# fdaPDE/fdaPDE-core

Hardware: AMD Instinct MI355X
Metric: DOF/s assemble+solve, 3D P1 Laplacian; SpMV achieved HBM GB/s vs peak (higher is better)
Workload: dtype f64

## Files before the change

fdapde-core_amd/csrc/dev_persist.hip:

```cpp
#include <hip/hip_runtime.h>
#include <hipcub/hipcub.hpp>

#include <algorithm>
#include <chrono>
#include <cstdint>
#include <string>
#include <vector>

#include "dev_persist.h"

namespace fdapde_hip {

namespace {

#define DP_CHK(expr)                                                          \
    do {                                                                      \
        hipError_t e__ = (expr);                                              \
        if (e__ != hipSuccess) {                                              \
            err = std::string(#expr) + ": " + hipGetErrorString(e__);         \
            return FDAPDE_EHIP;                                               \
        }                                                                     \
    } while (0)

struct Arena {
    std::vector<void*> slabs;
    char* cur = nullptr;
    size_t left = 0;
    static constexpr size_t kSlab = size_t(768) << 20;
    hipError_t take(size_t bytes, void** out) {
        bytes = (bytes + 255) & ~size_t(255);
        if (bytes > left) {
            const size_t sz = bytes > kSlab ? bytes : kSlab;
            void* p = nullptr;
            const hipError_t e = hipMalloc(&p, sz);
            if (e != hipSuccess) return e;
            slabs.push_back(p), cur = static_cast<char*>(p), left = sz;
        }
        *out = cur, cur += bytes, left -= bytes;
        return hipSuccess;
    }
    ~Arena() {
        for (void* p : slabs) (void)hipFree(p);
    }
};
thread_local Arena* t_arena = nullptr;
struct ArenaScope {
    Arena* prev;
    explicit ArenaScope(Arena* a) : prev(t_arena) { t_arena = a; }
    ~ArenaScope() { t_arena = prev; }
};
template <typename T> struct Tmp {
    T* p = nullptr;
    size_t n = 0;
    bool own = false;
    hipError_t alloc(size_t count) {
        reset();
        n = count;
        if (t_arena) return t_arena->take(sizeof(T) * (count ? count : 1), reinterpret_cast<void**>(&p));
        own = true;
        return hipMalloc(reinterpret_cast<void**>(&p), sizeof(T) * (count ? count : 1));
    }
    void reset() {
        if (p && own) (void)hipFree(p);
        p = nullptr, n = 0, own = false;
    }
    ~Tmp() { reset(); }
};
struct Scratch {
    void* p = nullptr;
    size_t n = 0;
    hipError_t need(size_t bytes) {
        if (bytes <= n) return hipSuccess;
        if (p) (void)hipFree(p);
        n = bytes + bytes / 4;
        return hipMalloc(&p, n);
    }
    ~Scratch() {
        if (p) (void)hipFree(p);
    }
};
inline unsigned grid_of(int64_t n) { return (unsigned)((n + 255) / 256); }

__device__ __forceinline__ int32_t wg_of_irow(const int32_t* wgs, int G, int64_t i) {
    int lo = 0, hi = G;
    while (hi - lo > 1) {
        const int mid = (lo + hi) >> 1;
        if (wgs[mid] <= i) lo = mid; else hi = mid;
    }
    return lo;
}
__global__ void k_balance_bounds(int G, int64_t nd, int64_t total, const int32_t* len_scan, const int32_t* irow_scan, int32_t* wgs) {
    const int g = blockIdx.x * blockDim.x + threadIdx.x;
    if (g > G) return;
    if (g == G) {
        wgs[G] = irow_scan[nd];
        return;
    }
    const int64_t target = (int64_t)g * total / G;
    int64_t lo = 0, hi = nd;
    while (lo < hi) {
        const int64_t mid = (lo + hi) >> 1;
        if ((int64_t)len_scan[mid] + 2 * (int64_t)irow_scan[mid] >= target) hi = mid; else lo = mid + 1;
    }
    wgs[g] = irow_scan[lo];
}
__global__ void k_wg_of(int64_t nd, const uint8_t* keep, const int32_t* irow, const int32_t* wgs, int G, int32_t* wg) {
    const int64_t d = (int64_t)blockIdx.x * blockDim.x + threadIdx.x;
    if (d < nd) wg[d] = keep[d] ? wg_of_irow(wgs, G, irow[d]) : -1;
}
__device__ __forceinline__ bool kept_entry(const uint8_t* keep, int32_t row, int32_t col) { return col != row && keep[col]; }

__global__ void k_keep_flags(int64_t nd, const uint8_t* bnd, int use_bnd, uint8_t* keep, int32_t* keep32) {
    const int64_t d = (int64_t)blockIdx.x * blockDim.x + threadIdx.x;
    if (d >= nd) return;
    const uint8_t k = (use_bnd && bnd[d]) ? 0 : 1;
    keep[d] = k, keep32[d] = k;
}
__global__ void k_row_lengths(int64_t nd, const int32_t* rowptr, const int32_t* colidx, const uint8_t* keep, int32_t* len) {
    const int64_t d = (int64_t)blockIdx.x * blockDim.x + threadIdx.x;
    if (d >= nd) return;
    int32_t n = 0;
    if (keep[d])
        for (int32_t k = rowptr[d]; k < rowptr[d + 1]; ++k) n += kept_entry(keep, (int32_t)d, colidx[k]);
    len[d] = n;
}
__global__ void k_sym_own_init(int64_t nd, const int32_t* rowptr, const int32_t* colidx, const uint8_t* keep, int32_t* own, const int32_t* irow,
                               int32_t* kept_dof) {
    const int64_t d = (int64_t)blockIdx.x * blockDim.x + threadIdx.x;
    if (d >= nd || !keep[d]) return;
    if (kept_dof) kept_dof[irow[d]] = (int32_t)d;
    for (int32_t k = rowptr[d]; k < rowptr[d + 1]; ++k) own[k] = persist_sym_owner((int32_t)d, colidx[k]) ? 1 : 0;
}
__global__ void k_sym_rows(int64_t nd, const int32_t* rowptr, const int32_t* colidx, const uint8_t* keep, const int32_t* wg, const int32_t* irow,
                           const int32_t* wgs, const int32_t* own, uint8_t* par, int32_t* up_k, int32_t* up_m, int32_t* up_loc) {
    const int64_t d = (int64_t)blockIdx.x * blockDim.x + threadIdx.x;
    if (d >= nd || !keep[d]) return;
    const int32_t g = wg[d], i = irow[d];
    int32_t len = 0, k_up = -1;
    for (int32_t k = rowptr[d]; k < rowptr[d + 1]; ++k) {
        const int32_t c = colidx[k];
        if (!kept_entry(keep, (int32_t)d, c)) continue;
        const bool inb = wg[c] == g;
        len += (!inb || own[k] != 0) ? 1 : 0;
        if (inb && c > (int32_t)d && k_up < 0) k_up = k;
    }
    par[i] = (uint8_t)(len & 1), up_k[i] = k_up;
    int32_t km = -1, loc = -1;
    if (k_up >= 0) {
        const int32_t c = colidx[k_up];
        int32_t lo = rowptr[c], hi = rowptr[c + 1];
        while (lo < hi) {
            const int32_t mid = (lo + hi) >> 1;
            if (colidx[mid] < (int32_t)d) lo = mid + 1; else hi = mid;
        }
        km = lo, loc = irow[c] - wgs[g];
    }
    up_m[i] = km, up_loc[i] = loc;
}
__global__ __launch_bounds__(256) void k_sym_walk(const int32_t* wgs, const uint8_t* par_g, const int32_t* up_k, const int32_t* up_m, const int32_t* up_loc,
                                                  int32_t* own) {
    extern __shared__ int32_t sw_lds[];
    const int g = blockIdx.x;
    const int32_t i0 = wgs[g], rows = wgs[g + 1] - i0;
    int32_t* up = sw_lds;
    uint8_t* par = reinterpret_cast<uint8_t*>(sw_lds + rows);
    for (int32_t i = threadIdx.x; i < rows; i += blockDim.x) up[i] = up_loc[i0 + i], par[i] = par_g[i0 + i];
    __syncthreads();
    if (threadIdx.x == 0)
        for (int32_t i = 0; i < rows; ++i) {
            const int32_t u = up[i];
            if ((par[i] & 1) && u >= 0) par[i] = 2, par[u] ^= 1;
        }
    __syncthreads();
    for (int32_t i = threadIdx.x; i < rows; i += blockDim.x)
        if (par[i] & 2) {
            const int32_t ku = up_k[i0 + i], km = up_m[i0 + i];
            own[ku] ^= 1, own[km] ^= 1;
        }
}
__global__ void k_row_lengths_sym(int64_t nd, const int32_t* rowptr, const int32_t* colidx, const uint8_t* keep, const int32_t* wg, const int32_t* own,
                                  int32_t* len) {
    const int64_t d = (int64_t)blockIdx.x * blockDim.x + threadIdx.x;
    if (d >= nd) return;
    int32_t n = 0;
    if (keep[d]) {
        const int32_t g = wg[d];
        for (int32_t k = rowptr[d]; k < rowptr[d + 1]; ++k) {
            const int32_t c = colidx[k];
            n += kept_entry(keep, (int32_t)d, c) && (wg[c] != g || own[k] != 0);
        }
    }
    len[d] = n;
}
__device__ __forceinline__ void wave_count_by_key(bool flag, int32_t key, int32_t* cnt) {
    unsigned long long todo = __ballot(flag);
    const int lane = (int)(threadIdx.x & 63);
    while (todo) {
        const int leader = __ffsll((long long)todo) - 1;
        const int32_t k0 = __shfl(key, leader);
        const unsigned long long same = __ballot(flag && key == k0);
        if (lane == leader) atomicAdd(&cnt[k0], (int32_t)__popcll(same));
        todo &= ~same;
    }
}
__global__ void k_row_halo(int64_t nd, const int32_t* rowptr, const int32_t* colidx, const uint8_t* keep, const int32_t* wg,
                           uint8_t* halo, int32_t* n_out, int32_t* wg_halo) {
    const int64_t d = (int64_t)blockIdx.x * blockDim.x + threadIdx.x;
    int32_t n = 0, g = -1;
    if (d < nd && keep[d]) {
        g = wg[d];
        for (int32_t k = rowptr[d]; k < rowptr[d + 1]; ++k) {
            const int32_t c = colidx[k];
            n += kept_entry(keep, (int32_t)d, c) && wg[c] != g;
        }
    }
    wave_count_by_key(n != 0, g, wg_halo);
    if (d < nd) halo[d] = n ? 1 : 0, n_out[d] = n;
}
__global__ void k_import_pairs(int64_t nd, const int32_t* rowptr, const int32_t* colidx, const uint8_t* keep, const int32_t* wg,
                               const int32_t* at, uint64_t* key) {
    const int64_t d = (int64_t)blockIdx.x * blockDim.x + threadIdx.x;
    if (d >= nd || !keep[d]) return;
    const int32_t g = wg[d];
    int32_t o = at[d];
    for (int32_t k = rowptr[d]; k < rowptr[d + 1]; ++k) {
        const int32_t c = colidx[k];
        if (kept_entry(keep, (int32_t)d, c) && wg[c] != g) key[o++] = ((uint64_t)(uint32_t)g << 32) | (uint32_t)c;
    }
}
__global__ void k_unique_flags(int64_t n, const uint64_t* key, int32_t* flag) {
    const int64_t i = (int64_t)blockIdx.x * blockDim.x + threadIdx.x;
    if (i < n) flag[i] = (i == 0 || key[i] != key[i - 1]) ? 1 : 0;
}
__global__ void k_compact_keys(int64_t n, const uint64_t* key, const int32_t* flag, const int32_t* pos, uint64_t* out) {
    const int64_t i = (int64_t)blockIdx.x * blockDim.x + threadIdx.x;
    if (i < n && flag[i]) out[pos[i]] = key[i];
}
__global__ void k_row_keys1(int64_t nd, const uint8_t* keep, const int32_t* irow, const int32_t* wg, const uint8_t* halo, const int32_t* len,
                            uint64_t* key, int32_t* val) {
    const int64_t d = (int64_t)blockIdx.x * blockDim.x + threadIdx.x;
    if (d >= nd || !keep[d]) return;
    const int32_t i = irow[d];
    key[i] = ((uint64_t)(uint32_t)wg[d] << 41) | ((uint64_t)halo[d] << 40) | ((uint64_t)(255 - len[d]) << 32) | (uint32_t)d;
    val[i] = (int32_t)d;
}
__global__ void k_row_keys2(int64_t n_int, const int32_t* dof_sorted, const int32_t* wgs, int G, int32_t sa, const uint8_t* halo, const int32_t* len,
                            uint64_t* key) {
    const int64_t p = (int64_t)blockIdx.x * blockDim.x + threadIdx.x;
    if (p >= n_int) return;
    const int32_t d = dof_sorted[p];
    const int64_t g = wg_of_irow(wgs, G, p), rank = p - wgs[g];
    const bool first = !halo[d] && rank < sa;
    const uint64_t payload = first ? (uint64_t)rank : (((uint64_t)(255 - len[d]) << 33) | ((uint64_t)halo[d] << 32) | (uint32_t)d);
    key[p] = ((uint64_t)g << 42) | ((uint64_t)(first ? 0 : 1) << 41) | payload;
}
__global__ void k_assign_slots(int64_t n_int, const int32_t* dof_sorted, const int32_t* wgs, int G, int32_t sa, int32_t S, const int32_t* wg_noimp, int32_t* slot_of,
                               int32_t* slot_dof) {
    const int64_t p = (int64_t)blockIdx.x * blockDim.x + threadIdx.x;
    if (p >= n_int) return;
    const int32_t d = dof_sorted[p];
    const int64_t g = wg_of_irow(wgs, G, p), i = p - wgs[g];
    const int32_t n_a = min(wg_noimp[g], sa);
    const int32_t slot = i < n_a ? (int32_t)i : sa + (int32_t)(i - n_a);
    slot_of[d] = slot;
    slot_dof[g * S + slot] = d;
}
__global__ void k_mark_exports(int64_t n_imp, const uint64_t* imp_key, uint8_t* is_exp) {
    const int64_t i = (int64_t)blockIdx.x * blockDim.x + threadIdx.x;
    if (i < n_imp) is_exp[imp_key[i] & 0xffffffffu] = 1;
}
__global__ void k_export_keys(int64_t nd, const uint8_t* is_exp, const int32_t* wg, const int32_t* slot_of, uint64_t* key, int32_t* val,
                              int32_t* n_out, int32_t* wg_exp) {
    const int64_t d = (int64_t)blockIdx.x * blockDim.x + threadIdx.x;
    const bool e = d < nd && is_exp[d];
    const int32_t g = e ? wg[d] : -1;
    const unsigned long long m = __ballot(e);
    if (m == 0) return;
    const int lane = (int)(threadIdx.x & 63), leader = __ffsll((long long)m) - 1;
    int32_t base = 0;
    if (lane == leader) base = atomicAdd(n_out, (int32_t)__popcll(m));
    base = __shfl(base, leader);
    if (e) {
        const int32_t o = base + (int32_t)__popcll(m & ((1ull << lane) - 1ull));
        key[o] = ((uint64_t)(uint32_t)g << 32) | (uint32_t)slot_of[d];
        val[o] = (int32_t)d;
    }
    wave_count_by_key(e, g, wg_exp);
}
__global__ void k_board_tables(int64_t n_board, const uint64_t* key_sorted, const int32_t* dof_sorted, uint16_t* exp_slot, int32_t* board_of) {
    const int64_t i = (int64_t)blockIdx.x * blockDim.x + threadIdx.x;
    if (i >= n_board) return;
    exp_slot[i] = (uint16_t)(key_sorted[i] & 0xffffu);
    board_of[dof_sorted[i]] = (int32_t)i;
}
__global__ void k_import_board_keys(int64_t n_imp, const uint64_t* imp_key, const int32_t* board_of, uint64_t* key, int32_t* wg_imp) {
    const int64_t i = (int64_t)blockIdx.x * blockDim.x + threadIdx.x;
    const bool in = i < n_imp;
    const uint64_t g = in ? imp_key[i] >> 32 : 0;
    if (in) key[i] = (g << 32) | (uint32_t)board_of[imp_key[i] & 0xffffffffu];
    wave_count_by_key(in, (int32_t)g, wg_imp);
}
__global__ void k_count_groups(int64_t n, const uint64_t* key, int32_t* count) {
    const int64_t i = (int64_t)blockIdx.x * blockDim.x + threadIdx.x;
    wave_count_by_key(i < n, i < n ? (int32_t)(key[i] >> 32) : 0, count);
}
__global__ void k_low32(int64_t n, const uint64_t* key, int32_t* out) {
    const int64_t i = (int64_t)blockIdx.x * blockDim.x + threadIdx.x;
    if (i < n) out[i] = (int32_t)(key[i] & 0xffffffffu);
}
__global__ void k_slice_pairs(int64_t n_sl, const int32_t* slot_dof, const int32_t* len, int32_t* pairs) {
    const int64_t q = (int64_t)blockIdx.x * blockDim.x + threadIdx.x;
    if (q >= n_sl) return;
    int32_t w = 0;
    for (int l = 0; l < 64; ++l) {
        const int32_t d = slot_dof[q * 64 + l];
        if (d >= 0) w = max(w, len[d]);
    }
    pairs[q] = (w + 1) / 2;
}
__global__ void k_slice_offsets(int G, int nsl, const int32_t* scan, int32_t* sl_off, int64_t* ell_off, int32_t* max_block) {
    const int64_t t = (int64_t)blockIdx.x * blockDim.x + threadIdx.x;
    if (t >= (int64_t)G * (nsl + 1)) return;
    const int64_t g = t / (nsl + 1), q = t - g * (nsl + 1);
    const int32_t base = scan[g * nsl];
    sl_off[t] = scan[g * nsl + q] - base;
    if (q == nsl) atomicMax(max_block, scan[g * nsl + nsl] - base);
    if (q == 0) ell_off[g] = (int64_t)base * 128;
    if (t == 0) ell_off[G] = (int64_t)scan[(int64_t)G * nsl] * 128;
}
__global__ void k_fill_ell(int64_t n_slots, int32_t S, int nsl, const int32_t* slot_dof, const int32_t* rowptr, const int32_t* colidx, const uint8_t* keep,
                           const int32_t* wg, const int32_t* slot_of, const int32_t* board_of, const int32_t* imp_off,
                           const int32_t* imp_pos, const int32_t* sl_off, const int64_t* ell_off, int sym, const int32_t* own, uint16_t* code, int32_t* src) {
    const int64_t t = (int64_t)blockIdx.x * blockDim.x + threadIdx.x;
    if (t >= n_slots) return;
    const int32_t d = slot_dof[t];
    if (d < 0 && !sym) return;
    const int64_t g = t / S;
    const int32_t s = (int32_t)(t - g * S), q = s / 64, l = s % 64;
    const int64_t base = ell_off[g] + (int64_t)sl_off[g * (nsl + 1) + q] * 128 + 2 * l;
    int32_t e = 0;
    for (int32_t k = d < 0 ? 0 : rowptr[d]; k < (d < 0 ? 0 : rowptr[d + 1]); ++k) {
        const int32_t c = colidx[k];
        if (!kept_entry(keep, d, c)) continue;
        if (sym && wg[c] == (int32_t)g && own[k] == 0) continue;
        const int64_t at = base + (int64_t)(e / 2) * 128 + (e & 1);
        src[at] = k;
        if (wg[c] == (int32_t)g) {
            code[at] = (uint16_t)slot_of[c];
        } else {
            int32_t lo = imp_off[g], hi = imp_off[g + 1];
            const int32_t b = board_of ? board_of[c] : c;
            while (lo < hi) {
                const int32_t mid = (lo + hi) >> 1;
                if (imp_pos[mid] < b) lo = mid + 1; else hi = mid;
            }
            code[at] = (uint16_t)(S + (lo - imp_off[g]));
        }
        ++e;
    }
    if (sym) {
        const int32_t e1 = 2 * (sl_off[g * (nsl + 1) + q + 1] - sl_off[g * (nsl + 1) + q]);
        for (; e < e1; ++e) code[base + (int64_t)(e / 2) * 128 + (e & 1)] = (uint16_t)s;
    }
}
__global__ void k_drop_list(int64_t nd, const uint8_t* keep, const int32_t* irow_scan, int32_t* drop) {
    const int64_t d = (int64_t)blockIdx.x * blockDim.x + threadIdx.x;
    if (d < nd && !keep[d]) drop[d - irow_scan[d]] = (int32_t)d;
}
__global__ void k_scatter_irow(int64_t nd, const uint8_t* keep, const int32_t* irow_scan, int32_t* irow) {
    const int64_t d = (int64_t)blockIdx.x * blockDim.x + threadIdx.x;
    if (d < nd) irow[d] = keep[d] ? irow_scan[d] : -1 - irow_scan[d];
}

template <typename K, typename V>
int sort_pairs(Scratch& sc, K* k_in, K* k_out, V* v_in, V* v_out, int64_t n, int end_bit, hipStream_t st, std::string& err) {
    size_t need = 0;
    DP_CHK(hipcub::DeviceRadixSort::SortPairs(nullptr, need, k_in, k_out, v_in, v_out, (int)n, 0, end_bit, st));
    DP_CHK(sc.need(need));
    DP_CHK(hipcub::DeviceRadixSort::SortPairs(sc.p, need, k_in, k_out, v_in, v_out, (int)n, 0, end_bit, st));
    return FDAPDE_OK;
}
template <typename K> int sort_keys(Scratch& sc, K* k_in, K* k_out, int64_t n, int end_bit, hipStream_t st, std::string& err) {
    size_t need = 0;
    DP_CHK(hipcub::DeviceRadixSort::SortKeys(nullptr, need, k_in, k_out, (int)n, 0, end_bit, st));
    DP_CHK(sc.need(need));
    DP_CHK(hipcub::DeviceRadixSort::SortKeys(sc.p, need, k_in, k_out, (int)n, 0, end_bit, st));
    return FDAPDE_OK;
}
template <typename In, typename Out> int exclusive_sum(Scratch& sc, In* in, Out* out, int64_t n, hipStream_t st, std::string& err) {
    size_t need = 0;
    DP_CHK(hipcub::DeviceScan::ExclusiveSum(nullptr, need, in, out, (int)n, st));
    DP_CHK(sc.need(need));
    DP_CHK(hipcub::DeviceScan::ExclusiveSum(sc.p, need, in, out, (int)n, st));
    return FDAPDE_OK;
}

}

void dev_persist_release(DevPersist* p) {
    if (!p) return;
    for (void* q : {(void*)p->slot_dof, (void*)p->sl_off, (void*)p->ell_src, (void*)p->exp_off, (void*)p->imp_off, (void*)p->imp_pos, (void*)p->ell_off,
                    (void*)p->ell_code, (void*)p->exp_slot, (void*)p->drop_dof})
        if (q) (void)hipFree(q);
    *p = DevPersist{};
}

int dev_build_persist_layout(int64_t nd, int32_t max_row, const int32_t* d_rowptr, const int32_t* d_colidx, const uint8_t* d_bnd, bool use_bnd,
                             int n_wg, int lds_entries, int blocked_rows, const int32_t* block_rows, int sym_mode, bool balance, void* stream, PersistLayout& pl, DevPersist* out,
                             std::string& err) {
    constexpr int T = kPersistT;
    hipStream_t st = static_cast<hipStream_t>(stream);
    if (n_wg < 1 || nd < 1 || max_row > 255) return FDAPDE_EUNSUPPORTED;
    const bool blocked = blocked_rows > 0;
    if (!blocked && n_wg > T) n_wg = T;
    Arena arena;
    ArenaScope arena_scope(&arena);
    Scratch sc;
    DevPersist o;
    struct Guard {
        DevPersist* p;
        bool armed = true;
        ~Guard() {
            if (armed) dev_persist_release(p);
        }
    } guard{&o};
    const bool dbg = std::getenv("FDAPDE_DEBUG_SETUP") != nullptr;
    auto t_ph = std::chrono::steady_clock::now();
    auto phase = [&](const char* name) {
        if (!dbg) return;
        (void)hipStreamSynchronize(st);
        const auto now = std::chrono::steady_clock::now();
        std::fprintf(stderr, "persist layout %-26s %8.2f ms\n", name, std::chrono::duration<double, std::milli>(now - t_ph).count());
        t_ph = now;
    };
    Tmp<uint8_t> keep, halo, is_exp;
    Tmp<int32_t> keep32, irow_scan, irow, len, n_imp_row, imp_at, wg_cnt;
    DP_CHK(keep.alloc((size_t)nd));
    DP_CHK(keep32.alloc((size_t)nd + 1));
    DP_CHK(irow_scan.alloc((size_t)nd + 1));
    DP_CHK(irow.alloc((size_t)nd));
    DP_CHK(len.alloc((size_t)nd + 1));
    DP_CHK(hipMemsetAsync(keep32.p + nd, 0, sizeof(int32_t), st));
    hipLaunchKernelGGL(k_keep_flags, dim3(grid_of(nd)), dim3(256), 0, st, nd, d_bnd, use_bnd ? 1 : 0, keep.p, keep32.p);
    if (int rc = exclusive_sum(sc, keep32.p, irow_scan.p, nd + 1, st, err)) return rc;
    hipLaunchKernelGGL(k_scatter_irow, dim3(grid_of(nd)), dim3(256), 0, st, nd, keep.p, irow_scan.p, irow.p);
    DP_CHK(hipMemsetAsync(len.p + nd, 0, sizeof(int32_t), st));
    hipLaunchKernelGGL(k_row_lengths, dim3(grid_of(nd)), dim3(256), 0, st, nd, d_rowptr, d_colidx, keep.p, len.p);
    Tmp<int32_t> len_scan;
    DP_CHK(len_scan.alloc((size_t)nd + 1));
    if (int rc = exclusive_sum(sc, len.p, len_scan.p, nd + 1, st, err)) return rc;
    int32_t h_nint = 0, h_nnz = 0;
    DP_CHK(hipMemcpyAsync(&h_nint, irow_scan.p + nd, sizeof(int32_t), hipMemcpyDeviceToHost, st));
    DP_CHK(hipMemcpyAsync(&h_nnz, len_scan.p + nd, sizeof(int32_t), hipMemcpyDeviceToHost, st));
    DP_CHK(hipStreamSynchronize(st));
    const int64_t n_int = h_nint, nnz_kept = h_nnz;
    if (n_int < 1) return FDAPDE_EUNSUPPORTED;
    const int64_t want = persist_want_workgroups(n_int, nnz_kept, lds_entries, blocked ? 0 : pl.single_rows);
    int G = (int)std::min<int64_t>(n_wg, want);
    if (blocked) G = (int)((n_int + blocked_rows - 1) / blocked_rows);
    if (G < 1) G = 1;
    if (G >= (1 << 20)) return FDAPDE_EUNSUPPORTED;
    int64_t rpw = (n_int + G - 1) / G;
    if (!blocked && block_rows == nullptr && rpw > (int64_t)kPersistRwide * T) return FDAPDE_EUNSUPPORTED;
    const bool sym = !blocked && persist_want_sym(sym_mode, nnz_kept, G, rpw) && rpw <= (int64_t)kPersistRmax * T;
    std::vector<int32_t> h_wgs;
    Tmp<int32_t> wgs, wg;
    bool uniform = true;
    if (block_rows != nullptr && !blocked) {
        G = n_wg;
        h_wgs.assign((size_t)G + 1, 0);
        rpw = 0;
        for (int g = 0; g < G; ++g) h_wgs[(size_t)g + 1] = h_wgs[(size_t)g] + block_rows[g], rpw = std::max<int64_t>(rpw, block_rows[g]);
        if (h_wgs[(size_t)G] != n_int) return FDAPDE_EINVAL;
        uniform = false;
    } else {
        G = (int)((n_int + rpw - 1) / rpw);
        DP_CHK(wgs.alloc((size_t)G + 1));
        if (balance && !blocked && G >= 2) {
            hipLaunchKernelGGL(k_balance_bounds, dim3((G + 256) / 256), dim3(256), 0, st, G, nd, nnz_kept + 2 * n_int, len_scan.p, irow_scan.p, wgs.p);
            h_wgs.assign((size_t)G + 1, 0);
            DP_CHK(hipMemcpyAsync(h_wgs.data(), wgs.p, sizeof(int32_t) * ((size_t)G + 1), hipMemcpyDeviceToHost, st));
            DP_CHK(hipStreamSynchronize(st));
            uniform = false;
            int64_t mx = 0;
            for (int g = 0; g < G; ++g) {
                if (h_wgs[(size_t)g + 1] <= h_wgs[(size_t)g]) uniform = true;
                mx = std::max<int64_t>(mx, h_wgs[(size_t)g + 1] - h_wgs[(size_t)g]);
            }
            const int64_t cap_rows = (int64_t)(rpw <= (int64_t)kPersistRmax * T ? kPersistRmax : kPersistRwide) * T;
            if (mx > cap_rows && rpw <= cap_rows) uniform = true;
            if (!uniform) rpw = mx;
        }
        if (uniform) {
            h_wgs.assign((size_t)G + 1, 0);
            for (int g = 0; g <= G; ++g) h_wgs[(size_t)g] = (int32_t)std::min<int64_t>(n_int, (int64_t)g * rpw);
        }
    }
    if (block_rows != nullptr && !blocked) DP_CHK(wgs.alloc((size_t)G + 1));
    DP_CHK(wg.alloc((size_t)nd));
    if (uniform || block_rows != nullptr) DP_CHK(hipMemcpyAsync(wgs.p, h_wgs.data(), sizeof(int32_t) * ((size_t)G + 1), hipMemcpyHostToDevice, st));
    hipLaunchKernelGGL(k_wg_of, dim3(grid_of(nd)), dim3(256), 0, st, nd, keep.p, irow.p, wgs.p, G, wg.p);
    phase("rows, workgroups");
    int64_t nnz_stored = nnz_kept;
    Tmp<int32_t> own;
    if (sym) {
        int32_t h_nnz_full = 0;
        DP_CHK(hipMemcpyAsync(&h_nnz_full, d_rowptr + nd, sizeof(int32_t), hipMemcpyDeviceToHost, st));
        DP_CHK(hipStreamSynchronize(st));
        DP_CHK(own.alloc((size_t)(h_nnz_full > 0 ? h_nnz_full : 1)));
        hipLaunchKernelGGL(k_sym_own_init, dim3(grid_of(nd)), dim3(256), 0, st, nd, d_rowptr, d_colidx, keep.p, own.p, irow.p, (int32_t*)nullptr);
        {
            Tmp<uint8_t> par;
            Tmp<int32_t> up_k, up_m, up_loc;
            DP_CHK(par.alloc((size_t)n_int));
            DP_CHK(up_k.alloc((size_t)n_int));
            DP_CHK(up_m.alloc((size_t)n_int));
            DP_CHK(up_loc.alloc((size_t)n_int));
            hipLaunchKernelGGL(k_sym_rows, dim3(grid_of(nd)), dim3(256), 0, st, nd, d_rowptr, d_colidx, keep.p, wg.p, irow.p, wgs.p, own.p, par.p, up_k.p, up_m.p,
                               up_loc.p);
            const size_t lds = (size_t)rpw * 5 + 16;
            hipLaunchKernelGGL(k_sym_walk, dim3(G), dim3(256), lds, st, wgs.p, par.p, up_k.p, up_m.p, up_loc.p, own.p);
            DP_CHK(hipGetLastError());
            if (!t_arena) DP_CHK(hipStreamSynchronize(st));
        }
        hipLaunchKernelGGL(k_row_lengths_sym, dim3(grid_of(nd)), dim3(256), 0, st, nd, d_rowptr, d_colidx, keep.p, wg.p, own.p, len.p);
        if (int rc = exclusive_sum(sc, len.p, len_scan.p, nd + 1, st, err)) return rc;
        DP_CHK(hipMemcpyAsync(&h_nnz, len_scan.p + nd, sizeof(int32_t), hipMemcpyDeviceToHost, st));
        DP_CHK(hipStreamSynchronize(st));
        nnz_stored = h_nnz;
    }
    phase("pair ownership (sym)");
    pl.n_drop = nd - n_int, pl.sym = sym;
    if (blocked) {
        DP_CHK(hipMalloc(reinterpret_cast<void**>(&o.drop_dof), sizeof(int32_t) * (size_t)(pl.n_drop ? pl.n_drop : 1)));
        hipLaunchKernelGGL(k_drop_list, dim3(grid_of(nd)), dim3(256), 0, st, nd, keep.p, irow_scan.p, o.drop_dof);
    }
    DP_CHK(halo.alloc((size_t)nd));
    DP_CHK(n_imp_row.alloc((size_t)nd + 1));
    DP_CHK(imp_at.alloc((size_t)nd + 1));
    DP_CHK(wg_cnt.alloc((size_t)3 * G));
    DP_CHK(hipMemsetAsync(wg_cnt.p, 0, sizeof(int32_t) * 3 * (size_t)G, st));
    DP_CHK(hipMemsetAsync(n_imp_row.p + nd, 0, sizeof(int32_t), st));
    hipLaunchKernelGGL(k_row_halo, dim3(grid_of(nd)), dim3(256), 0, st, nd, d_rowptr, d_colidx, keep.p, wg.p, halo.p, n_imp_row.p, wg_cnt.p);
    if (int rc = exclusive_sum(sc, n_imp_row.p, imp_at.p, nd + 1, st, err)) return rc;
    int32_t h_pairs = 0;
    std::vector<int32_t> h_cnt(3 * (size_t)G);
    DP_CHK(hipMemcpyAsync(&h_pairs, imp_at.p + nd, sizeof(int32_t), hipMemcpyDeviceToHost, st));
    DP_CHK(hipMemcpyAsync(h_cnt.data(), wg_cnt.p, sizeof(int32_t) * (size_t)G, hipMemcpyDeviceToHost, st));
    DP_CHK(hipStreamSynchronize(st));
    int32_t max_halo = 0;
    for (int g = 0; g < G; ++g) max_halo = std::max(max_halo, h_cnt[(size_t)g]);
    const int R = persist_rows_per_thread(rpw, max_halo, blocked, sym);
    if (R == 0) return FDAPDE_EUNSUPPORTED;
    const int S = R * T, nsl = S / 64, SA = blocked ? S : (R / 2) * T;
    pl.G = G, pl.R = R, pl.nsl = nsl, pl.n_int = n_int, pl.nnz = nnz_stored, pl.nnz_full = nnz_kept;
    Tmp<uint64_t> imp_key;
    int64_t n_imp = 0;
    {
        Tmp<uint64_t> k_a, k_s;
        Tmp<int32_t> flag, pos;
        DP_CHK(k_a.alloc((size_t)h_pairs));
        DP_CHK(k_s.alloc((size_t)h_pairs));
        DP_CHK(flag.alloc((size_t)h_pairs + 1));
        DP_CHK(pos.alloc((size_t)h_pairs + 1));
        hipLaunchKernelGGL(k_import_pairs, dim3(grid_of(nd)), dim3(256), 0, st, nd, d_rowptr, d_colidx, keep.p, wg.p, imp_at.p, k_a.p);
        if (h_pairs > 0) {
            if (int rc = sort_keys(sc, k_a.p, k_s.p, h_pairs, 53, st, err)) return rc;
            DP_CHK(hipMemsetAsync(flag.p + h_pairs, 0, sizeof(int32_t), st));
            hipLaunchKernelGGL(k_unique_flags, dim3(grid_of(h_pairs)), dim3(256), 0, st, (int64_t)h_pairs, k_s.p, flag.p);
            if (int rc = exclusive_sum(sc, flag.p, pos.p, (int64_t)h_pairs + 1, st, err)) return rc;
            int32_t h_n = 0;
            DP_CHK(hipMemcpyAsync(&h_n, pos.p + h_pairs, sizeof(int32_t), hipMemcpyDeviceToHost, st));
            DP_CHK(hipStreamSynchronize(st));
            n_imp = h_n;
            DP_CHK(imp_key.alloc((size_t)n_imp));
            hipLaunchKernelGGL(k_compact_keys, dim3(grid_of(h_pairs)), dim3(256), 0, st, (int64_t)h_pairs, k_s.p, flag.p, pos.p, imp_key.p);
            DP_CHK(hipStreamSynchronize(st));
        }
    }
    phase("import pairs");
    Tmp<int32_t> slot_of, dof1, wg_noimp;
    DP_CHK(slot_of.alloc((size_t)nd));
    DP_CHK(dof1.alloc((size_t)n_int));
    DP_CHK(hipMalloc(reinterpret_cast<void**>(&o.slot_dof), sizeof(int32_t) * (size_t)G * S));
    DP_CHK(hipMemsetAsync(o.slot_dof, 0xff, sizeof(int32_t) * (size_t)G * S, st));
    {
        Tmp<uint64_t> k_a, k_s;
        Tmp<int32_t> v_a, v_s;
        DP_CHK(k_a.alloc((size_t)n_int));
        DP_CHK(k_s.alloc((size_t)n_int));
        DP_CHK(v_a.alloc((size_t)n_int));
        DP_CHK(v_s.alloc((size_t)n_int));
        hipLaunchKernelGGL(k_row_keys1, dim3(grid_of(nd)), dim3(256), 0, st, nd, keep.p, irow.p, wg.p, halo.p, len.p, k_a.p, v_a.p);
        if (int rc = sort_pairs(sc, k_a.p, k_s.p, v_a.p, v_s.p, n_int, 62, st, err)) return rc;
        hipLaunchKernelGGL(k_row_keys2, dim3(grid_of(n_int)), dim3(256), 0, st, n_int, v_s.p, wgs.p, G, (int32_t)SA, halo.p, len.p, k_a.p);
        if (int rc = sort_pairs(sc, k_a.p, k_s.p, v_s.p, dof1.p, n_int, 63, st, err)) return rc;
        std::vector<int32_t> h_noimp((size_t)G);
        for (int g = 0; g < G; ++g)
            h_noimp[(size_t)g] = (h_wgs[(size_t)g + 1] - h_wgs[(size_t)g]) - (blocked ? 0 : h_cnt[(size_t)g]);
        DP_CHK(wg_noimp.alloc((size_t)G));
        DP_CHK(hipMemcpyAsync(wg_noimp.p, h_noimp.data(), sizeof(int32_t) * (size_t)G, hipMemcpyHostToDevice, st));
        hipLaunchKernelGGL(k_assign_slots, dim3(grid_of(n_int)), dim3(256), 0, st, n_int, dof1.p, wgs.p, G, (int32_t)SA, (int32_t)S, wg_noimp.p, slot_of.p,
                           o.slot_dof);
        DP_CHK(hipStreamSynchronize(st));
    }
    phase("slots");
    Tmp<int32_t> board_of;
    DP_CHK(board_of.alloc((size_t)nd));
    DP_CHK(is_exp.alloc((size_t)nd));
    DP_CHK(hipMemsetAsync(is_exp.p, 0, (size_t)nd, st));
    if (n_imp > 0 && !blocked) hipLaunchKernelGGL(k_mark_exports, dim3(grid_of(n_imp)), dim3(256), 0, st, n_imp, imp_key.p, is_exp.p);
    int64_t n_board = 0;
    if (!blocked) {
        Tmp<uint64_t> k_a, k_s;
        Tmp<int32_t> v_a, v_s, cnt;
        const int64_t cap = n_imp > 0 ? n_imp : 1;
        DP_CHK(k_a.alloc((size_t)cap));
        DP_CHK(k_s.alloc((size_t)cap));
        DP_CHK(v_a.alloc((size_t)cap));
        DP_CHK(v_s.alloc((size_t)cap));
        DP_CHK(cnt.alloc(1));
        DP_CHK(hipMemsetAsync(cnt.p, 0, sizeof(int32_t), st));
        hipLaunchKernelGGL(k_export_keys, dim3(grid_of(nd)), dim3(256), 0, st, nd, is_exp.p, wg.p, slot_of.p, k_a.p, v_a.p, cnt.p, wg_cnt.p + G);
        int32_t h_nb = 0;
        DP_CHK(hipMemcpyAsync(&h_nb, cnt.p, sizeof(int32_t), hipMemcpyDeviceToHost, st));
        DP_CHK(hipStreamSynchronize(st));
        n_board = h_nb;
        DP_CHK(hipMalloc(reinterpret_cast<void**>(&o.exp_slot), sizeof(uint16_t) * (size_t)(n_board ? n_board : 1)));
        if (n_board > 0) {
            if (int rc = sort_pairs(sc, k_a.p, k_s.p, v_a.p, v_s.p, n_board, 42, st, err)) return rc;
            hipLaunchKernelGGL(k_board_tables, dim3(grid_of(n_board)), dim3(256), 0, st, n_board, k_s.p, v_s.p, o.exp_slot, board_of.p);
        }
        DP_CHK(hipStreamSynchronize(st));
    }
    DP_CHK(hipMalloc(reinterpret_cast<void**>(&o.imp_pos), sizeof(int32_t) * (size_t)(n_imp ? n_imp : 1)));
    if (blocked) {
        DP_CHK(hipMalloc(reinterpret_cast<void**>(&o.exp_slot), sizeof(uint16_t)));
        if (n_imp > 0) {
            hipLaunchKernelGGL(k_low32, dim3(grid_of(n_imp)), dim3(256), 0, st, n_imp, imp_key.p, o.imp_pos);
            hipLaunchKernelGGL(k_count_groups, dim3(grid_of(n_imp)), dim3(256), 0, st, n_imp, imp_key.p, wg_cnt.p + 2 * G);
        }
    } else if (n_imp > 0) {
        Tmp<uint64_t> k_a, k_s;
        DP_CHK(k_a.alloc((size_t)n_imp));
        DP_CHK(k_s.alloc((size_t)n_imp));
        hipLaunchKernelGGL(k_import_board_keys, dim3(grid_of(n_imp)), dim3(256), 0, st, n_imp, imp_key.p, board_of.p, k_a.p, wg_cnt.p + 2 * G);
        if (int rc = sort_keys(sc, k_a.p, k_s.p, n_imp, 42, st, err)) return rc;
        hipLaunchKernelGGL(k_low32, dim3(grid_of(n_imp)), dim3(256), 0, st, n_imp, k_s.p, o.imp_pos);
        DP_CHK(hipStreamSynchronize(st));
    }
    DP_CHK(hipMemcpyAsync(h_cnt.data() + G, wg_cnt.p + G, sizeof(int32_t) * 2 * (size_t)G, hipMemcpyDeviceToHost, st));
    DP_CHK(hipStreamSynchronize(st));
    std::vector<int32_t> h_exp_off((size_t)G + 1, 0), h_imp_off((size_t)G + 1, 0);
    pl.max_exp = pl.max_imp = 0;
    for (int g = 0; g < G; ++g) {
        h_exp_off[(size_t)g + 1] = h_exp_off[(size_t)g] + h_cnt[(size_t)G + g], pl.max_exp = std::max(pl.max_exp, h_cnt[(size_t)G + g]);
        h_imp_off[(size_t)g + 1] = h_imp_off[(size_t)g] + h_cnt[(size_t)2 * G + g], pl.max_imp = std::max(pl.max_imp, h_cnt[(size_t)2 * G + g]);
    }
    pl.n_board = n_board, pl.n_imp = n_imp;
    if (S + pl.max_imp > 65535) return FDAPDE_EUNSUPPORTED;
    DP_CHK(hipMalloc(reinterpret_cast<void**>(&o.exp_off), sizeof(int32_t) * ((size_t)G + 1)));
    DP_CHK(hipMalloc(reinterpret_cast<void**>(&o.imp_off), sizeof(int32_t) * ((size_t)G + 1)));
    DP_CHK(hipMemcpyAsync(o.exp_off, h_exp_off.data(), sizeof(int32_t) * ((size_t)G + 1), hipMemcpyHostToDevice, st));
    DP_CHK(hipMemcpyAsync(o.imp_off, h_imp_off.data(), sizeof(int32_t) * ((size_t)G + 1), hipMemcpyHostToDevice, st));
    phase("boards");
    const int64_t n_sl = (int64_t)G * nsl;
    Tmp<int32_t> pairs, pscan, max_block;
    DP_CHK(pairs.alloc((size_t)n_sl + 1));
    DP_CHK(pscan.alloc((size_t)n_sl + 1));
    DP_CHK(max_block.alloc(1));
    DP_CHK(hipMemsetAsync(pairs.p + n_sl, 0, sizeof(int32_t), st));
    DP_CHK(hipMemsetAsync(max_block.p, 0, sizeof(int32_t), st));
    hipLaunchKernelGGL(k_slice_pairs, dim3(grid_of(n_sl)), dim3(256), 0, st, n_sl, o.slot_dof, len.p, pairs.p);
    if (int rc = exclusive_sum(sc, pairs.p, pscan.p, n_sl + 1, st, err)) return rc;
    DP_CHK(hipMalloc(reinterpret_cast<void**>(&o.sl_off), sizeof(int32_t) * (size_t)G * (nsl + 1)));
    DP_CHK(hipMalloc(reinterpret_cast<void**>(&o.ell_off), sizeof(int64_t) * ((size_t)G + 1)));
    hipLaunchKernelGGL(k_slice_offsets, dim3(grid_of((int64_t)G * (nsl + 1))), dim3(256), 0, st, G, nsl, pscan.p, o.sl_off, o.ell_off, max_block.p);
    int32_t h_total = 0, h_maxb = 0;
    DP_CHK(hipMemcpyAsync(&h_total, pscan.p + n_sl, sizeof(int32_t), hipMemcpyDeviceToHost, st));
    DP_CHK(hipMemcpyAsync(&h_maxb, max_block.p, sizeof(int32_t), hipMemcpyDeviceToHost, st));
    DP_CHK(hipStreamSynchronize(st));
    pl.n_entries = (int64_t)h_total * 128;
    pl.max_block = (int64_t)h_maxb * 128;
    const size_t n_alloc = (size_t)pl.n_entries + 256;
    DP_CHK(hipMalloc(reinterpret_cast<void**>(&o.ell_code), sizeof(uint16_t) * n_alloc));
    DP_CHK(hipMalloc(reinterpret_cast<void**>(&o.ell_src), sizeof(int32_t) * n_alloc));
    DP_CHK(hipMemsetAsync(o.ell_code, 0, sizeof(uint16_t) * n_alloc, st));
    DP_CHK(hipMemsetAsync(o.ell_src, 0xff, sizeof(int32_t) * n_alloc, st));
    hipLaunchKernelGGL(k_fill_ell, dim3(grid_of((int64_t)G * S)), dim3(256), 0, st, (int64_t)G * S, (int32_t)S, nsl, o.slot_dof, d_rowptr, d_colidx, keep.p, wg.p,
                       slot_of.p, blocked ? (const int32_t*)nullptr : board_of.p, o.imp_off, o.imp_pos, o.sl_off, o.ell_off, sym ? 1 : 0, sym ? own.p : (const int32_t*)nullptr, o.ell_code, o.ell_src);
    DP_CHK(hipGetLastError());
    DP_CHK(hipStreamSynchronize(st));
    phase("sliced ELL");
    guard.armed = false;
    *out = o;
    return FDAPDE_OK;
}

void dev_persist_preload() {
    hipFuncAttributes attr;
    (void)hipFuncGetAttributes(&attr, reinterpret_cast<const void*>(&k_keep_flags));
    (void)hipGetLastError();
}

}
```

fdapde-core_amd/csrc/host_persist.cpp:

```cpp
#include <algorithm>
#include <cstddef>
#include <cstdint>
#include <numeric>
#include <thread>
#include <vector>

#include "internal.h"

namespace fdapde_hip {

namespace {

template <typename F> void for_each_wg(int G, F&& fn) {
    unsigned nt = std::thread::hardware_concurrency();
    nt = nt < 1 ? 1 : (nt > 16 ? 16 : nt);
    if ((unsigned)G < nt) nt = (unsigned)G;
    if (nt <= 1) {
        for (int g = 0; g < G; ++g) fn(g);
        return;
    }
    std::vector<std::thread> th;
    for (unsigned t = 0; t < nt; ++t)
        th.emplace_back([&, t] {
            for (int g = (int)t; g < G; g += (int)nt) fn(g);
        });
    for (auto& x : th) x.join();
}

}

int host_build_persist_layout(const HostSpace& hs, bool use_bnd, int n_wg, int lds_entries, PersistLayout& pl, const int32_t* block_rows, int sym_mode, bool balance,
                              const int32_t* ghost_order, bool allow_late) {
    constexpr int T = kPersistT;
    const int64_t nd = hs.n_dofs;
    if (n_wg < 1 || nd < 1) return FDAPDE_EUNSUPPORTED;
    if (n_wg > T) n_wg = T;
    auto dropped = [&](int64_t d) { return use_bnd && hs.dof_bnd_i[(size_t)d] != 0; };
    std::vector<int32_t> irow_dof;
    irow_dof.reserve((size_t)nd);
    auto ghost = [&](int64_t d) { return ghost_order != nullptr && ghost_order[(size_t)d] >= 0; };
    for (int64_t d = 0; d < nd; ++d)
        if (!dropped(d) && !ghost(d)) irow_dof.push_back((int32_t)d);
    const int64_t n_int = (int64_t)irow_dof.size();
    if (n_int < 1) return FDAPDE_EUNSUPPORTED;
    auto kept = [&](int64_t row, int32_t col) { return col != row && !dropped(col); };
    int64_t nnz_kept = 0;
    for (int64_t i = 0; i < n_int; ++i) {
        const int32_t d = irow_dof[(size_t)i];
        for (int32_t k = hs.rowptr_i[(size_t)d]; k < hs.rowptr_i[(size_t)d + 1]; ++k) nnz_kept += kept(d, hs.colidx_i[(size_t)k]);
    }
    const int64_t want = persist_want_workgroups(n_int, nnz_kept, lds_entries, ghost_order != nullptr ? 0 : pl.single_rows);
    int G = (int)std::min<int64_t>(n_wg, want);
    if (G < 1) G = 1;
    int64_t rpw = (n_int + G - 1) / G;
    if (block_rows == nullptr && rpw > (int64_t)kPersistRwide * T) return FDAPDE_EUNSUPPORTED;
    const bool sym = persist_want_sym(sym_mode, nnz_kept, G, rpw) && rpw <= (int64_t)kPersistRmax * T;
    std::vector<int64_t> wgs;
    if (block_rows != nullptr) {
        G = n_wg;
        wgs.assign((size_t)G + 1, 0);
        rpw = 0;
        for (int g = 0; g < G; ++g) wgs[(size_t)g + 1] = wgs[(size_t)g] + block_rows[g], rpw = std::max<int64_t>(rpw, block_rows[g]);
        if (wgs[(size_t)G] != n_int) return FDAPDE_EINVAL;
    } else {
        G = (int)((n_int + rpw - 1) / rpw);
        bool uniform = true;
        if (balance && G >= 2) {
            const int64_t total = nnz_kept + 2 * n_int;
            wgs.assign((size_t)G + 1, n_int);
            int64_t cost = 0;
            int g = 0;
            for (int64_t i = 0; i < n_int; ++i) {
                while (g < G && cost >= (int64_t)g * total / G) wgs[(size_t)g++] = i;
                const int32_t d = irow_dof[(size_t)i];
                int64_t len = 0;
                for (int32_t k = hs.rowptr_i[(size_t)d]; k < hs.rowptr_i[(size_t)d + 1]; ++k) len += kept(d, hs.colidx_i[(size_t)k]);
                cost += len + 2;
            }
            uniform = false;
            int64_t mx = 0;
            for (int q = 0; q < G; ++q) {
                if (wgs[(size_t)q + 1] <= wgs[(size_t)q]) uniform = true;
                mx = std::max(mx, wgs[(size_t)q + 1] - wgs[(size_t)q]);
            }
            const int64_t cap_rows = (int64_t)(rpw <= (int64_t)kPersistRmax * T ? kPersistRmax : kPersistRwide) * T;
            if (mx > cap_rows && rpw <= cap_rows) uniform = true;
            if (!uniform) rpw = mx;
        }
        if (uniform) {
            wgs.assign((size_t)G + 1, 0);
            for (int g = 0; g <= G; ++g) wgs[(size_t)g] = std::min<int64_t>(n_int, (int64_t)g * rpw);
        }
    }
    std::vector<int32_t> wg_of((size_t)nd, -1), slot_of((size_t)nd, -1);
    for (int g = 0; g < G; ++g)
        for (int64_t i = wgs[(size_t)g]; i < wgs[(size_t)g + 1]; ++i) wg_of[(size_t)irow_dof[(size_t)i]] = g;

    std::vector<uint8_t> own;
    if (sym) {
        own.assign((size_t)hs.nnz, 0);
        for (int64_t i = 0; i < n_int; ++i) {
            const int32_t d = irow_dof[(size_t)i];
            for (int32_t k = hs.rowptr_i[(size_t)d]; k < hs.rowptr_i[(size_t)d + 1]; ++k) own[(size_t)k] = persist_sym_owner(d, hs.colidx_i[(size_t)k]) ? 1 : 0;
        }
        for_each_wg(G, [&](int g) {
            for (int64_t i = wgs[(size_t)g]; i < wgs[(size_t)g + 1]; ++i) {
                const int32_t d = irow_dof[(size_t)i];
                int32_t len = 0, k_up = -1;
                for (int32_t k = hs.rowptr_i[(size_t)d]; k < hs.rowptr_i[(size_t)d + 1]; ++k) {
                    const int32_t c = hs.colidx_i[(size_t)k];
                    if (!kept(d, c)) continue;
                    const bool in_block = wg_of[(size_t)c] == g;
                    len += !in_block || own[(size_t)k];
                    if (in_block && c > d && k_up < 0) k_up = k;
                }
                if ((len & 1) == 0 || k_up < 0) continue;
                const int32_t c = hs.colidx_i[(size_t)k_up];
                const int32_t* lo = &hs.colidx_i[(size_t)hs.rowptr_i[(size_t)c]];
                const int32_t* hi = &hs.colidx_i[(size_t)hs.rowptr_i[(size_t)c + 1]];
                const int32_t k_mirror = (int32_t)(std::lower_bound(lo, hi, d) - &hs.colidx_i[0]);
                own[(size_t)k_up] ^= 1, own[(size_t)k_mirror] ^= 1;
            }
        });
    }

    struct Key { int32_t halo, len, dof; };
    std::vector<std::vector<Key>> wg_rows((size_t)G);
    std::vector<std::vector<int32_t>> imports((size_t)G);
    std::vector<int32_t> row_len((size_t)nd, 0), n_halo((size_t)G, 0);
    for_each_wg(G, [&](int g) {
        const int64_t i0 = wgs[(size_t)g], i1 = wgs[(size_t)g + 1];
        std::vector<Key>& rows = wg_rows[(size_t)g];
        rows.reserve((size_t)(i1 - i0));
        std::vector<int32_t>& imp = imports[(size_t)g];
        for (int64_t i = i0; i < i1; ++i) {
            const int32_t d = irow_dof[(size_t)i];
            int32_t len = 0, halo = 0;
            for (int32_t k = hs.rowptr_i[(size_t)d]; k < hs.rowptr_i[(size_t)d + 1]; ++k) {
                const int32_t c = hs.colidx_i[(size_t)k];
                if (!kept(d, c)) continue;
                if (sym && wg_of[(size_t)c] == g && !own[(size_t)k]) continue;
                ++len;
                if (wg_of[(size_t)c] != g) halo = 1, imp.push_back(c);
            }
            row_len[(size_t)d] = len;
            rows.push_back({halo, len, d});
            n_halo[(size_t)g] += halo;
        }
        std::sort(imp.begin(), imp.end());
        imp.erase(std::unique(imp.begin(), imp.end()), imp.end());
    });
    const int32_t max_halo = *std::max_element(n_halo.begin(), n_halo.end());
    const int R = persist_rows_per_thread(rpw, max_halo, allow_late, sym);
    if (R == 0) return FDAPDE_EUNSUPPORTED;
    const int S = R * T, nsl = S / 64, SA = (R / 2) * T;
    pl.G = G, pl.R = R, pl.nsl = nsl, pl.n_int = n_int, pl.sym = sym, pl.nnz_full = nnz_kept;
    pl.wg_late.assign((size_t)G, 0);
    if (allow_late)
        for (int g = 0; g < G; ++g) pl.wg_late[(size_t)g] = n_halo[(size_t)g] > SA ? 1 : 0;

    pl.slot_dof.assign((size_t)G * S, -1);
    for_each_wg(G, [&](int g) {
        std::vector<Key>& rows = wg_rows[(size_t)g];
        std::sort(rows.begin(), rows.end(), [](const Key& a, const Key& b) {
            if (a.halo != b.halo) return a.halo < b.halo;
            if (a.len != b.len) return a.len > b.len;
            return a.dof < b.dof;
        });
        const bool late = allow_late && n_halo[(size_t)g] > SA;
        const size_t n_noimp = rows.size() - (size_t)n_halo[(size_t)g], n_a = late ? rows.size() : std::min<size_t>(n_noimp, (size_t)SA);
        if (late) std::stable_sort(rows.begin(), rows.end(), [](const Key& a, const Key& b) { return a.len > b.len; });
        else std::stable_sort(rows.begin() + (std::ptrdiff_t)n_a, rows.end(), [](const Key& a, const Key& b) { return a.len > b.len; });
        for (size_t i = 0; i < rows.size(); ++i) {
            const size_t s = i < n_a ? i : (size_t)SA + (i - n_a);
            pl.slot_dof[(size_t)g * S + s] = rows[i].dof;
            slot_of[(size_t)rows[i].dof] = (int32_t)s;
        }
        rows = {};
    });

    std::vector<uint8_t> is_exp((size_t)nd, 0);
    for (int g = 0; g < G; ++g)
        for (int32_t d : imports[(size_t)g]) is_exp[(size_t)d] = 1;
    pl.exp_off.assign((size_t)G + 1, 0);
    std::vector<int32_t> board_of((size_t)nd, -1);
    pl.exp_slot.clear();
    pl.max_exp = 0;
    for (int g = 0; g < G; ++g) {
        int32_t cnt = 0;
        for (int s = 0; s < S; ++s) {
            const int32_t d = pl.slot_dof[(size_t)g * S + s];
            if (d < 0 || !is_exp[(size_t)d]) continue;
            board_of[(size_t)d] = pl.exp_off[(size_t)g] + cnt;
            pl.exp_slot.push_back((uint16_t)s);
            ++cnt;
        }
        pl.exp_off[(size_t)g + 1] = pl.exp_off[(size_t)g] + cnt;
        pl.max_exp = std::max(pl.max_exp, cnt);
    }
    pl.n_board = pl.exp_off[(size_t)G];
    pl.ghost_needed.clear();
    if (ghost_order != nullptr) {
        for (int64_t d = 0; d < nd; ++d)
            if (ghost(d) && is_exp[(size_t)d]) pl.ghost_needed.push_back((int32_t)d);
        std::sort(pl.ghost_needed.begin(), pl.ghost_needed.end(), [&](int32_t a, int32_t b) { return ghost_order[(size_t)a] < ghost_order[(size_t)b]; });
        for (size_t k = 0; k < pl.ghost_needed.size(); ++k) board_of[(size_t)pl.ghost_needed[k]] = (int32_t)(pl.n_board + (int64_t)k);
    }
    pl.imp_off.assign((size_t)G + 1, 0);
    pl.max_imp = 0;
    for (int g = 0; g < G; ++g) {
        std::vector<int32_t>& imp = imports[(size_t)g];
        std::sort(imp.begin(), imp.end(), [&](int32_t a, int32_t b) { return board_of[(size_t)a] < board_of[(size_t)b]; });
        pl.imp_off[(size_t)g + 1] = pl.imp_off[(size_t)g] + (int32_t)imp.size();
        pl.max_imp = std::max(pl.max_imp, (int32_t)imp.size());
    }
    if (S + pl.max_imp > 65535) return FDAPDE_EUNSUPPORTED;
    pl.imp_pos.resize((size_t)pl.imp_off[(size_t)G]);
    pl.n_imp = pl.imp_off[(size_t)G];
    for (int g = 0; g < G; ++g)
        for (size_t h = 0; h < imports[(size_t)g].size(); ++h)
            pl.imp_pos[(size_t)pl.imp_off[(size_t)g] + h] = board_of[(size_t)imports[(size_t)g][h]];

    pl.sl_off.assign((size_t)G * (nsl + 1), 0);
    pl.ell_off.assign((size_t)G + 1, 0);
    for (int g = 0; g < G; ++g) {
        int32_t off = 0;
        for (int q = 0; q < nsl; ++q) {
            int32_t w = 0;
            for (int l = 0; l < 64; ++l) {
                const int32_t d = pl.slot_dof[(size_t)g * S + (size_t)q * 64 + l];
                if (d >= 0) w = std::max(w, row_len[(size_t)d]);
            }
            pl.sl_off[(size_t)g * (nsl + 1) + q] = off;
            off += (w + 1) / 2;
        }
        pl.sl_off[(size_t)g * (nsl + 1) + nsl] = off;
        pl.ell_off[(size_t)g + 1] = pl.ell_off[(size_t)g] + (int64_t)off * 128;
    }
    pl.n_entries = pl.ell_off[(size_t)G];
    pl.ell_code.assign((size_t)pl.n_entries, 0);
    pl.ell_src.assign((size_t)pl.n_entries, -1);
    std::vector<int64_t> nnz_wg((size_t)G, 0);
    for_each_wg(G, [&](int g) {
        const std::vector<int32_t>& imp = imports[(size_t)g];
        std::vector<int32_t> by_dof(imp.size());
        std::iota(by_dof.begin(), by_dof.end(), 0);
        std::sort(by_dof.begin(), by_dof.end(), [&](int32_t a, int32_t b) { return imp[(size_t)a] < imp[(size_t)b]; });
        auto import_index = [&](int32_t dof) {
            size_t lo = 0, hi = by_dof.size();
            while (lo < hi) {
                const size_t mid = (lo + hi) / 2;
                if (imp[(size_t)by_dof[mid]] < dof) lo = mid + 1;
                else hi = mid;
            }
            return by_dof[lo];
        };
        int64_t nz = 0;
        for (int s = 0; s < S; ++s) {
            const int32_t d = pl.slot_dof[(size_t)g * S + s];
            if (d < 0 && !sym) continue;
            const int q = s / 64, l = s % 64;
            const int64_t base = pl.ell_off[(size_t)g] + (int64_t)pl.sl_off[(size_t)g * (nsl + 1) + q] * 128 + 2 * l;
            int32_t e = 0;
            for (int32_t k = d < 0 ? 0 : hs.rowptr_i[(size_t)d]; k < (d < 0 ? 0 : hs.rowptr_i[(size_t)d + 1]); ++k) {
                const int32_t c = hs.colidx_i[(size_t)k];
                if (!kept(d, c)) continue;
                if (sym && wg_of[(size_t)c] == g && !own[(size_t)k]) continue;
                const int64_t at = base + (int64_t)(e / 2) * 128 + (e & 1);
                pl.ell_src[(size_t)at] = k;
                pl.ell_code[(size_t)at] = (uint16_t)(wg_of[(size_t)c] == g ? slot_of[(size_t)c] : S + import_index(c));
                ++e, ++nz;
            }
            if (sym) {
                const int32_t e1 = 2 * (pl.sl_off[(size_t)g * (nsl + 1) + q + 1] - pl.sl_off[(size_t)g * (nsl + 1) + q]);
                for (; e < e1; ++e) pl.ell_code[(size_t)(base + (int64_t)(e / 2) * 128 + (e & 1))] = (uint16_t)s;
            }
        }
        nnz_wg[(size_t)g] = nz;
    });
    pl.nnz = std::accumulate(nnz_wg.begin(), nnz_wg.end(), (int64_t)0);
    if (ghost_order != nullptr) pl.wg_of = std::move(wg_of), pl.slot_of = std::move(slot_of);
    return FDAPDE_OK;
}

}
```

Measured before the change: 112.8 million.

## Reorder symmetric sliced-ELL entries per lane to reduce LDS bank conflicts

```diff
diff --git a/fdapde-core_amd/csrc/dev_persist.hip b/fdapde-core_amd/csrc/dev_persist.hip
--- a/fdapde-core_amd/csrc/dev_persist.hip
+++ b/fdapde-core_amd/csrc/dev_persist.hip
@@ -8,6 +8,7 @@
 #include <vector>
 
 #include "dev_persist.h"
+#include "persist_order.h"
 
 namespace fdapde_hip {
 
@@ -362,6 +363,54 @@
         const int32_t e1 = 2 * (sl_off[g * (nsl + 1) + q + 1] - sl_off[g * (nsl + 1) + q]);
         for (; e < e1; ++e) code[base + (int64_t)(e / 2) * 128 + (e & 1)] = (uint16_t)s;
     }
+}
+__global__ __launch_bounds__(256) void k_order_ell(int64_t n_groups, int32_t S, int nsl, const int32_t* sl_off, const int64_t* ell_off, uint16_t* code, int32_t* src) {
+    __shared__ PersistOrderScratch scr[4];
+    const int wv = threadIdx.x / 64, lane = threadIdx.x % 64;
+    const int64_t t = (int64_t)blockIdx.x * 4 + wv;
+    if (t >= n_groups) return;
+    const int64_t gq = t >> 1, g = gq / nsl;
+    const int q = (int)(gq - g * nsl), half = (int)(t & 1);
+    const int32_t* slo = &sl_off[g * (nsl + 1) + q];
+    const int E = 2 * (slo[1] - slo[0]);
+    if (E <= 1 || E > kOrderMaxSteps) return;
+    uint16_t* cb = code + ell_off[g] + (int64_t)slo[0] * 128;
+    int32_t* sb = src + ell_off[g] + (int64_t)slo[0] * 128;
+    PersistOrderScratch& sc = scr[wv];
+    for (int i = lane; i < E * 32; i += 64) sc.cr[i / 32][i % 32] = 0, sc.ca[i / 32][i % 32] = 0;
+    __builtin_amdgcn_fence(__ATOMIC_SEQ_CST, "workgroup");
+    for (int sweep = 0; sweep < 2; ++sweep)
+        for (int i = 0; i < 32; ++i) {
+            const int l = 32 * half + i;
+            const int at = (lane >> 1) * 128 + 2 * l + (lane & 1);
+            const unsigned c = lane < E ? cb[at] : 0u;
+            const int32_t k = lane < E ? sb[at] : -1;
+            const int a = (int)(c & 31u), b = c < (unsigned)S ? (int)(c & 31u) : (l & 31);
+            if (sweep > 0 && lane < E) --sc.cr[lane][a], --sc.ca[lane][b];
+            __builtin_amdgcn_fence(__ATOMIC_SEQ_CST, "wavefront");
+            uint32_t used = 0;
+            int mine = 0;
+            for (int e = 0; e < E; ++e) {
+                const int ae = __builtin_amdgcn_readlane(a, e), be = __builtin_amdgcn_readlane(b, e);
+                const bool free_step = lane < E && !((used >> lane) & 1u);
+                const int cost = free_step ? sc.cr[lane][ae] + sc.ca[lane][be] : 0;
+                unsigned long long cand = __ballot(free_step);
+                for (int bit = 6; bit >= 0; --bit) {
+                    const unsigned long long z = cand & __ballot(((cost >> bit) & 1) == 0);
+                    if (z) cand = z;
+                }
+                const int best = __ffsll((long long)cand) - 1;
+                if (lane == e) mine = best;
+                used |= 1u << best;
+                if (lane == 0) ++sc.cr[best][ae], ++sc.ca[best][be];
+                __builtin_amdgcn_fence(__ATOMIC_SEQ_CST, "wavefront");
+            }
+            if (lane < E) {
+                const int to = (mine >> 1) * 128 + 2 * l + (mine & 1);
+                cb[to] = (uint16_t)c, sb[to] = k;
+            }
+            __builtin_amdgcn_fence(__ATOMIC_SEQ_CST, "workgroup");
+        }
 }
 __global__ void k_drop_list(int64_t nd, const uint8_t* keep, const int32_t* irow_scan, int32_t* drop) {
     const int64_t d = (int64_t)blockIdx.x * blockDim.x + threadIdx.x;
@@ -689,6 +738,11 @@
     DP_CHK(hipMemsetAsync(o.ell_src, 0xff, sizeof(int32_t) * n_alloc, st));
     hipLaunchKernelGGL(k_fill_ell, dim3(grid_of((int64_t)G * S)), dim3(256), 0, st, (int64_t)G * S, (int32_t)S, nsl, o.slot_dof, d_rowptr, d_colidx, keep.p, wg.p,
                        slot_of.p, blocked ? (const int32_t*)nullptr : board_of.p, o.imp_off, o.imp_pos, o.sl_off, o.ell_off, sym ? 1 : 0, sym ? own.p : (const int32_t*)nullptr, o.ell_code, o.ell_src);
+    if (sym) {
+        const int64_t n_groups = (int64_t)G * nsl * 2;
+        hipLaunchKernelGGL(k_order_ell, dim3((unsigned)((n_groups + 3) / 4)), dim3(256), 0, st, n_groups, (int32_t)S, nsl, o.sl_off,
+                           o.ell_off, o.ell_code, o.ell_src);
+    }
     DP_CHK(hipGetLastError());
     DP_CHK(hipStreamSynchronize(st));
     phase("sliced ELL");
diff --git a/fdapde-core_amd/csrc/host_persist.cpp b/fdapde-core_amd/csrc/host_persist.cpp
--- a/fdapde-core_amd/csrc/host_persist.cpp
+++ b/fdapde-core_amd/csrc/host_persist.cpp
@@ -6,6 +6,7 @@
 #include <vector>
 
 #include "internal.h"
+#include "persist_order.h"
 
 namespace fdapde_hip {
 
@@ -276,6 +277,14 @@
                 for (; e < e1; ++e) pl.ell_code[(size_t)(base + (int64_t)(e / 2) * 128 + (e & 1))] = (uint16_t)s;
             }
         }
+        if (sym) {
+            PersistOrderScratch sc;
+            for (int q = 0; q < nsl; ++q) {
+                const int32_t* slo = &pl.sl_off[(size_t)g * (nsl + 1) + q];
+                const int64_t base = pl.ell_off[(size_t)g] + (int64_t)slo[0] * 128;
+                for (int h = 0; h < 2; ++h) persist_order_half(&pl.ell_code[(size_t)base], &pl.ell_src[(size_t)base], 2 * (slo[1] - slo[0]), S, h, sc);
+            }
+        }
         nnz_wg[(size_t)g] = nz;
     });
     pl.nnz = std::accumulate(nnz_wg.begin(), nnz_wg.end(), (int64_t)0);
diff --git a/fdapde-core_amd/csrc/persist_order.h b/fdapde-core_amd/csrc/persist_order.h
--- /dev/null
+++ b/fdapde-core_amd/csrc/persist_order.h
@@ -0,0 +1,53 @@
+#pragma once
+#include <cstdint>
+
+#if defined(__HIPCC__)
+#define FDAPDE_PO_HD __host__ __device__
+#else
+#define FDAPDE_PO_HD
+#endif
+
+namespace fdapde_hip {
+
+constexpr int kOrderMaxSteps = 32;
+
+struct PersistOrderScratch {
+    uint8_t cr[kOrderMaxSteps][32];
+    uint8_t ca[kOrderMaxSteps][32];
+};
+
+FDAPDE_PO_HD inline void persist_order_half(uint16_t* code, int32_t* src, int E, int S, int half, PersistOrderScratch& sc) {
+    if (E <= 1 || E > kOrderMaxSteps) return;
+    for (int t = 0; t < E; ++t)
+        for (int r = 0; r < 32; ++r) sc.cr[t][r] = 0, sc.ca[t][r] = 0;
+    auto at = [](int e, int l) { return (e >> 1) * 128 + 2 * l + (e & 1); };
+    auto res_read = [](unsigned c) { return (int)(c & 31u); };
+    auto res_add = [S](unsigned c, int l) { return c < (unsigned)S ? (int)(c & 31u) : (l & 31); };
+    for (int sweep = 0; sweep < 2; ++sweep) {
+        for (int i = 0; i < 32; ++i) {
+            const int l = 32 * half + i;
+            uint16_t c[kOrderMaxSteps], nc[kOrderMaxSteps];
+            int32_t k[kOrderMaxSteps], nk[kOrderMaxSteps];
+            for (int e = 0; e < E; ++e) {
+                c[e] = code[at(e, l)], k[e] = src[at(e, l)];
+                if (sweep > 0) --sc.cr[e][res_read(c[e])], --sc.ca[e][res_add(c[e], l)];
+            }
+            uint32_t used = 0;
+            for (int e = 0; e < E; ++e) {
+                const int a = res_read(c[e]), b = res_add(c[e], l);
+                int best = -1, best_cost = 1 << 30;
+                for (int t = 0; t < E; ++t) {
+                    if ((used >> t) & 1u) continue;
+                    const int cost = sc.cr[t][a] + sc.ca[t][b];
+                    if (cost < best_cost) best_cost = cost, best = t;
+                }
+                used |= 1u << best;
+                ++sc.cr[best][a], ++sc.ca[best][b];
+                nc[best] = c[e], nk[best] = k[e];
+            }
+            for (int e = 0; e < E; ++e) code[at(e, l)] = nc[e], src[at(e, l)] = nk[e];
+        }
+    }
+}
+
+}
```

Measured after the change: 114.0 million, median of 6. +1.1%, better.
